# GassiusODude/spectral_analyzer

Hardware: NVIDIA B200
Metric: spectrogram Msamples/s (cf32, 1024-pt FFT) (higher is better)
Workload: dtype f32

## Files before the change

### spectral_analyzer_b200/csrc/engine.cu

```cuda
#include "engine_internal.h"

#include <algorithm>
#include <cmath>
#include <cstdarg>
#include <cstdio>
#include <cstdlib>
#include <cstring>
#include <cerrno>
#include <fcntl.h>
#include <sys/stat.h>
#include <unistd.h>

namespace sa {

#ifndef SA_LARGE_DUAL_DEFAULT
#define SA_LARGE_DUAL_DEFAULT 0
#endif
constexpr bool kLargeDualDefault = SA_LARGE_DUAL_DEFAULT != 0;
constexpr uint64_t kLargeDualWsMb = 48;

CopyPool::CopyPool(int workers) {
    for (int i = 0; i < workers; i++) threads_.emplace_back([this] { worker(); });
}
CopyPool::~CopyPool() {
// ... 265 lines not shown
    return fn;
}

int Engine::launch_spectrogram_large(const void* d_iq, uint64_t n_samples, const sa_spectrogram_params& p, int prec,
                                     const SpecArgs& base, void* d_out, cudaStream_t stream, int ws) {
    (void)d_iq; (void)n_samples; (void)d_out;
    const int dk = dtype_kind(p.dtype);
    const int win = (prec == SA_PREC_F64) ? 1 : (p.window != SA_WIN_RECT ? 1 : 0);
    const LargeKernelInfo* k = find_large_kernel(prec, (int)p.nfft, dk, win);
    if (!k) return set_error(SA_ERR_UNSUPPORTED, "no kernel for nfft %u precision %s dtype %d", p.nfft,
                             prec == SA_PREC_F64 ? "f64" : "f32", p.dtype);
    LargeArgs a;
    memset(&a, 0, sizeof(a));
    a.s = base;
    const SpecKernelInfo* k1 = find_spec_kernel(prec, k->n1, DK_CF32, 1, 0);
    const SpecKernelInfo* k2 = find_spec_kernel(prec, k->n2, DK_CF32, 1, 0);
    if (!k1 || !k2) return set_error(SA_ERR_UNSUPPORTED, "sub-transform plans %d / %d missing", k->n1, k->n2);
    int rc = twiddle_table(*k1, &a.s.twiddle);
    if (rc) return rc;
    rc = twiddle_table(*k2, &a.tw2);
    if (rc) return rc;
    rc = root_table((int)p.nfft, prec, &a.tw_n);
    if (rc) return rc;
    if (win) { rc = window_table(p.window, (int)p.nfft, prec, &a.s.window); if (rc) return rc; }
    const size_t elem = (prec == SA_PREC_F64) ? 16 : 8;
    const uint64_t per_frame = (uint64_t)p.nfft * elem;
    void* args[] = { &a };
    cudaError_t e;
    const char* onchip_env = getenv("SA_LARGE_ONCHIP");
    const bool use_onchip = onchip_env ? atoi(onchip_env) != 0 : false;
    const uint64_t iq_b = (uint64_t)sa_bytes_per_iq(p.dtype);
    const bool aligned = ((uintptr_t)d_iq % 16 == 0) && ((p.start_sample * iq_b) % 16 == 0) && ((p.hop * iq_b) % 16 == 0);
    if (k->fn_cluster && use_onchip && aligned) {
        auto it = occupancy.find(k->fn_cluster);
        int n_clusters = 0;
        cudaLaunchConfig_t cfg;
        memset(&cfg, 0, sizeof(cfg));
        cudaLaunchAttribute attr[1];
        attr[0].id = cudaLaunchAttributeClusterDimension;
        attr[0].val.clusterDim.x = kLargeCluster; attr[0].val.clusterDim.y = 1; attr[0].val.clusterDim.z = 1;
        cfg.blockDim = dim3(k->cta_cluster);
        cfg.dynamicSmemBytes = k->smem_cluster;
        cfg.stream = stream;
        cfg.attrs = attr; cfg.numAttrs = 1;
        if (it == occupancy.end()) {
            e = cudaFuncSetAttribute(k->fn_cluster, cudaFuncAttributeMaxDynamicSharedMemorySize, (int)k->smem_cluster);
            if (e != cudaSuccess) return cuda_fail(e, "on-chip four-step smem attribute");
            cfg.gridDim = dim3(kLargeCluster * num_sms);
            e = cudaOccupancyMaxActiveClusters(&n_clusters, k->fn_cluster, &cfg);
            if (e != cudaSuccess || n_clusters < 1) { cudaGetLastError(); n_clusters = 0; }
            occupancy[k->fn_cluster] = n_clusters;
        } else {
            n_clusters = it->second;
        }
        const uint64_t first_end = p.start_sample + p.nfft;
        const uint64_t n_read = n_samples >= first_end ? std::min<uint64_t>(p.n_frames, (n_samples - first_end) / p.hop + 1) : 0;
        CUtensorMap tmap;
        bool have_map = false;
        if (n_clusters > 0 && n_read > 0 && encode_tiled_fn()) {
            const cuuint64_t e8 = iq_b / 8;
            const cuuint64_t gdim[3] = { (cuuint64_t)k->n2 * e8, (cuuint64_t)k->n1, (cuuint64_t)n_read };
            const cuuint64_t gstr[2] = { (cuuint64_t)k->n2 * iq_b, (cuuint64_t)p.hop * iq_b };
            const cuuint32_t box[3] = { (cuuint32_t)(kLargeC * e8), (cuuint32_t)k->n1, 1 };
            const cuuint32_t estr[3] = { 1, 1, 1 };
            void* gaddr = (char*)const_cast<void*>(d_iq) + p.start_sample * iq_b;
            have_map = gstr[1] < (1ull << 40) &&
                       encode_tiled_fn()(&tmap, CU_TENSOR_MAP_DATA_TYPE_UINT64, 3, gaddr, gdim, gstr, box, estr, CU_TENSOR_MAP_INTERLEAVE_NONE,
                                         CU_TENSOR_MAP_SWIZZLE_NONE, CU_TENSOR_MAP_L2_PROMOTION_L2_256B,
                                         CU_TENSOR_MAP_FLOAT_OOB_FILL_NONE) == CUDA_SUCCESS;
        }
        if (have_map) {
            const uint64_t use = std::min<uint64_t>((uint64_t)n_clusters, p.n_frames);
            a.ws = nullptr;
#if SA_ONCHIP_PROF
            rc = ensure_scratch(ws, (size_t)use * kLargeCluster * 16 * sizeof(long long));
            if (rc) return rc;
            a.ws = scratch[ws];
#endif
            a.frame0 = 0;
            cfg.gridDim = dim3((unsigned)(use * kLargeCluster));
            void* cargs[] = { &a, &tmap };
            e = cudaLaunchKernelExC(&cfg, k->fn_cluster, cargs);
            if (e != cudaSuccess) return cuda_fail(e, "launch large_onchip_kernel");
            launches++;
// ... 138 lines not shown
            cudaLaunchConfig_t cfg;
            memset(&cfg, 0, sizeof(cfg));
            cfg.stream = st; cfg.attrs = attr; cfg.numAttrs = 1;
            cfg.gridDim = dim3(k->n2 / kLargeC, nf); cfg.blockDim = dim3(k->cta_cols); cfg.dynamicSmemBytes = k->smem_cols;
            e = cudaLaunchKernelExC(&cfg, k->fn_cols, args);
            if (e != cudaSuccess) return cuda_fail(e, "launch large_cols_kernel");
            cfg.gridDim = dim3(k->n1 / kLargeC, nf); cfg.blockDim = dim3(k->cta_rows); cfg.dynamicSmemBytes = k->smem_rows;
            e = cudaLaunchKernelExC(&cfg, k->fn_rows, args);
            if (e != cudaSuccess) return cuda_fail(e, "launch large_rows_kernel");
            launches += 2;
            continue;
        }
        e = cudaLaunchKernel(k->fn_cols, dim3(k->n2 / kLargeC, nf), dim3(k->cta_cols), args, k->smem_cols, st);
        if (e != cudaSuccess) return cuda_fail(e, "launch large_cols_kernel");
        e = cudaLaunchKernel(k->fn_rows, dim3(k->n1 / kLargeC, nf), dim3(k->cta_rows), args, k->smem_rows, st);
        if (e != cudaSuccess) return cuda_fail(e, "launch large_rows_kernel");
        launches += 2;
    }
    {
        static const char* const dkn[] = { "cf32", "ci16", "c8", "cf64" };
        char nm[160];
        snprintf(nm, sizeof(nm), "large_cols_kernel+large_rows_kernel<%s,%dx%d,%s,%s>", prec == SA_PREC_F64 ? "double" : "float",
                 k->n1, k->n2, dkn[dk], win ? "window" : "rect");
        last_kernel = nm;
    }
    if (dual) {
        e = cudaEventRecord(large_ev[ai][1], large_aux[ai]);
        if (e == cudaSuccess) e = cudaStreamWaitEvent(stream, large_ev[ai][1], 0);
        if (e != cudaSuccess) return cuda_fail(e, "four-step join");
    }
    return SA_OK;
}

int Engine::kernel_grid(const void* fn, int cta, size_t smem, int* blocks_per_sm) {
    auto it = occupancy.find(fn);
    if (it != occupancy.end()) { *blocks_per_sm = it->second; return SA_OK; }
    cudaError_t e = cudaFuncSetAttribute(fn, cudaFuncAttributeMaxDynamicSharedMemorySize, (int)smem);
    if (e != cudaSuccess) return cuda_fail(e, "cudaFuncSetAttribute(smem)");
    int nb = 0;
    e = cudaOccupancyMaxActiveBlocksPerMultiprocessor(&nb, fn, cta, smem);
    if (e != cudaSuccess) return cuda_fail(e, "occupancy query");
    if (nb < 1) return set_error(SA_ERR_CUDA, "kernel does not fit on an SM (smem %zu)", smem);
    occupancy[fn] = nb;
    *blocks_per_sm = nb;
    return SA_OK;
}

int dtype_kind(int dtype) {
    switch (dtype) {
        case SA_CF32: return DK_CF32;
        case SA_CI16: return DK_CI16;
        case SA_CU8:
        case SA_CI8:  return DK_C8;
        case SA_CF64: return DK_CF64;
        default:      return -1;
    }
}

void fill_load_params(LoadParams& lp, const void* base, int dtype, int big_endian) {
    lp.base = base;
    lp.swap = big_endian ? 1 : 0;
    lp.c8_flip = (dtype == SA_CI8) ? 0x80808080u : 0u;
    lp.c8_off = (dtype == SA_CI8) ? 1.0f : 127.5f / 128.0f;
    lp.c8_c = 256.0f + lp.c8_off;
}

static bool is_pow2(uint64_t x) { return x && !(x & (x - 1)); }

static bool strict_zero(const sa_spectrogram_params& p) {
    return p.strict_reference && (p.dtype == SA_CF64 || p.dtype == SA_DT_OTHER);
}
uint64_t spec_bytes_per_iq(const sa_spectrogram_params& p) {
    if (p.dtype == SA_DT_OTHER) return p.strict_reference ? 8 : 0;
    return (uint64_t)sa_bytes_per_iq(p.dtype);
}

// ... 93 lines not shown
    }
    if (p.nfft > 16384 || (prec == SA_PREC_F64 && p.nfft > 8192))
        return launch_spectrogram_large(d_iq, n_samples, p, prec, a, d_out, stream, ws);
    const uint64_t iq_b = (uint64_t)sa_bytes_per_iq(p.dtype);
    const bool aligned = ((uintptr_t)d_iq % 16 == 0) && ((p.start_sample * iq_b) % 16 == 0) && ((p.hop * iq_b) % 16 == 0);
    static const bool no_tma = getenv("SA_NO_TMA") != nullptr;
    static const bool no_mid = getenv("SA_NO_MID") != nullptr;
    const SpecKernelInfo* k = (aligned && !no_tma) ? find_spec_kernel(prec, (int)p.nfft, dk, win, 1) : nullptr;
    static const char* r64_env = getenv("SA_R64");
    const bool use_r64 = r64_env ? (strcmp(r64_env, "all") == 0) : (dk == DK_CF32 || dk == DK_CI16);
    if (!k && aligned && use_r64 && !pool_mode && prec == SA_PREC_F32 && p.nfft == 4096) k = find_spec_kernel(prec, 4096, dk, win, 4);
    const char* split_env = getenv("SA_SPLIT");
    const bool use_split = split_env ? atoi(split_env) != 0 : false;
    if (!k && aligned && use_split && !pool_mode && prec == SA_PREC_F32 && p.nfft == 2048) k = find_spec_kernel(prec, 2048, dk, win, 5);
    if (!k && aligned && !no_mid) {
        static const char* pf_env = getenv("SA_MID_PF");
        const bool pf = pf_env ? (strcmp(pf_env, "all") == 0) : (p.nfft != 8192);
        if (pf) k = find_spec_kernel(prec, (int)p.nfft, dk, win, 3);
        if (!k) k = find_spec_kernel(prec, (int)p.nfft, dk, win, 2);
    }
    if (!k) k = find_spec_kernel(prec, (int)p.nfft, dk, win, 0);
    if (!k) return set_error(SA_ERR_UNSUPPORTED, "no kernel for nfft %u precision %s dtype %d", p.nfft,
                             prec == SA_PREC_F64 ? "f64" : "f32", p.dtype);
    int rc;
    if (k->tma >= 2) {
        rc = mid_t1_table(k->n, &a.twiddle);
        if (rc) return rc;
        rc = root_table(k->n, prec, &a.aux);
    } else {
        rc = twiddle_table(*k, &a.twiddle);
    }
    if (rc) return rc;
    if (win) { rc = window_table(p.window, (int)p.nfft, prec, &a.window); if (rc) return rc; }
    int bps = 0;
    rc = kernel_grid(k->fn, k->cta, k->smem, &bps);
    if (rc) return rc;
    const long long n_blocks = ((long long)p.n_frames + k->fpc - 1) / k->fpc;
    const long long max_grid = (long long)bps * num_sms;
    const unsigned grid = (unsigned)std::min<long long>(n_blocks, max_grid);
    void* args[] = { &a };
    cudaError_t e = cudaLaunchKernel(k->fn, dim3(grid), dim3(k->cta), args, k->smem, stream);
    if (e != cudaSuccess) return cuda_fail(e, "launch spectrogram_kernel");
    launches++;
    {
        static const char* const fam[] = { "spectrogram_kernel", "spectrogram_tma_kernel", "spectrogram_mid_kernel",
                                           "spectrogram_mid_kernel(prefetch)", "spectrogram_r64_kernel", "spectrogram_split_kernel" };
        static const char* const dkn[] = { "cf32", "ci16", "c8", "cf64" };
        char nm[128];
        snprintf(nm, sizeof(nm), "%s<%s,%d,%s,%s>", fam[k->tma], prec == SA_PREC_F64 ? "double" : "float", k->n, dkn[k->dk],
                 k->win ? "window" : "rect");
        last_kernel = nm;
    }
    return SA_OK;
}

static CopyPool* make_copy_pool() {
    const char* ev = getenv("SA_COPY_THREADS");
    const unsigned hw = std::thread::hardware_concurrency();
    int n = ev ? atoi(ev) : (int)std::min(32u, std::max(2u, hw));
    return new CopyPool(std::max(1, n - 1));
}

void Engine::host_copy(void* dst, const void* src, size_t bytes) {
    if (bytes < (4u << 20)) { memcpy(dst, src, bytes); return; }
    if (!copy_pool) copy_pool = make_copy_pool();
    copy_pool->copy(dst, src, bytes);
}

bool Engine::host_read(void* dst, int fd, uint64_t off, size_t bytes) {
    if (!copy_pool) copy_pool = make_copy_pool();
    return copy_pool->read(dst, fd, off, bytes);
}

int Engine::ensure_staging(Slot& s, size_t in_bytes, size_t out_bytes) {
// ... 364 lines not shown
```

### spectral_analyzer_b200/csrc/fft_core.cuh

```cuda
#pragma once
#include <cuda_runtime.h>
#include <stdint.h>

#ifndef SA_WARPS_1WPF
#define SA_WARPS_1WPF 16
#endif
#ifndef SA_CTA_1WPF
#define SA_CTA_1WPF 512
#endif
#ifndef SA_CTA_F64
#define SA_CTA_F64 512
#endif
#ifndef SA_WIN_SMEM_MAX_TPF
#define SA_WIN_SMEM_MAX_TPF 128
#endif
#ifndef SA_TW_SMEM_MAX_TPF
#define SA_TW_SMEM_MAX_TPF 32
#endif
#ifndef SA_PACKED_SMALL_RADIX
#define SA_PACKED_SMALL_RADIX 0
#endif
#ifndef SA_TW_RECURRENCE
#define SA_TW_RECURRENCE 1
#endif
// ... 272 lines not shown
SA_PLAN(double,   64,  8, 2,  8,  8,  1, 1)
SA_PLAN(double,  128, 16, 2, 16,  8,  1, 1)
SA_PLAN(double,  256, 16, 2, 16, 16,  1, 1)
SA_PLAN(double,  512, 16, 3, 16, 16,  2, 1)
SA_PLAN(double, 1024, 16, 3, 16, 16,  4, 1)
SA_PLAN(double, 2048, 16, 3, 16, 16,  8, 1)
SA_PLAN(double, 4096, 16, 3, 16, 16, 16, 1)
SA_PLAN(double, 8192, 16, 4, 16, 16, 16, 2)
#undef SA_PLAN

template <typename T, int N> struct Geo {
    using PL = Plan<T, N>;
    static constexpr int P = PL::P;
    static constexpr int TPF = N / P;
    static constexpr int CTA = (sizeof(T) == 4 && TPF <= 32) ? SA_CTA_1WPF
                             : (sizeof(T) == 8 && TPF <= 32) ? SA_CTA_F64 : (TPF > 128 ? TPF : 128);
    static constexpr int FPC = CTA / TPF;
    static constexpr int MINB = (sizeof(T) == 4 && TPF <= 32) ? SA_WARPS_1WPF * 32 / CTA : 512 / CTA;
    static constexpr int WROW = P + 2;
    static constexpr bool WIN_SMEM = TPF <= SA_WIN_SMEM_MAX_TPF;
    static constexpr size_t WIN_BYTES = WIN_SMEM ? (size_t)TPF * WROW * sizeof(T) : 0;
    static constexpr int R0 = PL::radix(0);
    static constexpr int PADW = sizeof(T) == 4 ? 2 : 1;
    static constexpr int SM_ELEMS = N + (N / R0) * PADW;
    static constexpr size_t SMEM_BYTES = (size_t)FPC * SM_ELEMS * sizeof(cpx<T>);
    static constexpr bool TW_REC = SA_TW_RECURRENCE && sizeof(T) == 4 && PL::NP == 2 && PL::radix(1) == P;
    static constexpr bool TW_SMEM = TPF <= SA_TW_SMEM_MAX_TPF;
    static constexpr size_t TW_BYTES = TW_SMEM ? (size_t)(PL::NP - 1) * N * sizeof(cpx<T>) : 0;
    static constexpr size_t EXTRA_WIN_OFF = SMEM_BYTES + TW_BYTES;
    static constexpr int TW_ELEMS = (PL::NP - 1) * N;
    __host__ __device__ static constexpr int ns(int pass) { int r = 1; for (int i = 0; i < pass; i++) r *= PL::radix(i); return r; }
};

template <int R0, int PADW> __device__ __forceinline__ int pad_idx(int i) { return i + (i / R0) * PADW; }

template <int TPF, bool BSYNC = false> __device__ __forceinline__ void frame_sync() {
    if constexpr (TPF <= 32 && !BSYNC) __syncwarp(); else __syncthreads();
}

template <typename T, int N, int PASS, bool WIN, bool REC, bool BSYNC = false>
__device__ __forceinline__ void fft_pass(cpx<T> (&v)[Plan<T, N>::P], const int t, cpx<T>* __restrict__ sm,
                                         const cpx<T>* __restrict__ tw, const T* __restrict__ win,
                                         const TwSeed<T>& seed) {
    using G = Geo<T, N>;
    using PL = Plan<T, N>;
    constexpr int P = G::P, TPF = G::TPF, R = PL::radix(PASS), S = P / R, NS = G::ns(PASS);
    if constexpr (PASS == 0) {
        RadixAll<T, R, S, P, WIN ? MUL_REAL : MUL_NONE, false, 0>::run(v, win, nullptr, TPF, seed);
    } else {
        const TwPair<T>* twp = reinterpret_cast<const TwPair<T>*>(tw) + (size_t)(PASS - 1) * (N / 2) + t;
        if constexpr (REC && G::TW_REC) RadixAll<T, R, S, P, MUL_REC, false, 0>::run(v, nullptr, nullptr, TPF, seed);
        else RadixAll<T, R, S, P, MUL_CPX, G::TW_SMEM, 0>::run(v, nullptr, twp, TPF, seed);
    }
    if constexpr (PASS + 1 < PL::NP) {
        frame_sync<TPF, BSYNC>();
#pragma unroll
        for (int s = 0; s < S; s++) {
            const int j = t + TPF * s;
            const int base = (j / NS) * (NS * R) + (j % NS);
            if constexpr (NS == 1 && sizeof(T) == 4) {
                float4* dst = reinterpret_cast<float4*>(sm + pad_idx<G::R0, G::PADW>(base));
#pragma unroll
                for (int m = 0; m < R; m += 2)
                    dst[m / 2] = make_float4(v[s + m * S].x, v[s + m * S].y, v[s + (m + 1) * S].x, v[s + (m + 1) * S].y);
            } else {
#pragma unroll
                for (int m = 0; m < R; m++) sm[pad_idx<G::R0, G::PADW>(base + m * NS)] = v[s + m * S];
            }
        }
        frame_sync<TPF, BSYNC>();
#pragma unroll
        for (int q = 0; q < P; q++) v[q] = sm[pad_idx<G::R0, G::PADW>(t + TPF * q)];
    }
}

template <typename T, int N>
__device__ __forceinline__ TwSeed<T> load_tw_seed(const cpx<T>* __restrict__ tw, const int t) {
    using G = Geo<T, N>;
    TwSeed<T> s;
    s.om = mk2<T>((T)1, (T)0); s.oh = s.om;
    if constexpr (G::TW_REC) {
        const TwPair<T>* p = reinterpret_cast<const TwPair<T>*>(tw);
        s.om = ldg_tw<false>(p + 1 * G::TPF + t).lo;
        s.oh = ldg_tw<false>(p + 0 * G::TPF + t).hi;
    }
    return s;
}

template <typename T, int N, bool WIN, bool REC = false, bool BSYNC = false>
__device__ __forceinline__ void fft_frame(cpx<T> (&v)[Plan<T, N>::P], const int t, cpx<T>* __restrict__ sm,
                                          const cpx<T>* __restrict__ tw, const T* __restrict__ win,
                                          const TwSeed<T>& seed) {
    using PL = Plan<T, N>;
    fft_pass<T, N, 0, WIN, REC, BSYNC>(v, t, sm, tw, win, seed);
    if constexpr (PL::NP > 1) fft_pass<T, N, 1, WIN, REC, BSYNC>(v, t, sm, tw, win, seed);
    if constexpr (PL::NP > 2) fft_pass<T, N, 2, WIN, REC, BSYNC>(v, t, sm, tw, win, seed);
    if constexpr (PL::NP > 3) fft_pass<T, N, 3, WIN, REC, BSYNC>(v, t, sm, tw, win, seed);
}

}
```

### spectral_analyzer_b200/csrc/spectrogram_kernel.cuh

```cuda
#pragma once
#include "decode.cuh"

#ifndef SA_POOL_EPILOGUE
#define SA_POOL_EPILOGUE 1
#endif
#ifndef SA_STORE_STREAMING
#define SA_STORE_STREAMING 0
#endif

namespace sa {

enum { OUT_F32_DB = 0, OUT_F64_DB = 1, OUT_RGBA8 = 2 };
enum { DBM_MAG_1E10 = 0, DBM_POWER = 1 };

struct SpecArgs {
    LoadParams  lp;
    long long   n_samples;
    long long   start_sample;
    long long   hop;
    long long   n_frames;
    const void* window;
    const void* twiddle;
    const void* aux;
    void*       out;
    int         out_kind;
    int         db_mode;
    double      eof_fill;
    float       cmap_bias;
    float       inv_range;
    int         cmap;
    int         pool_mode;
    float       pool_eof;
    long long   pool_fpc;
    unsigned long long pool_magic;
};
__device__ __forceinline__ long long pool_column(const SpecArgs& a, long long frame) {
    return a.pool_magic ? (long long)__umul64hi((unsigned long long)frame, a.pool_magic) : frame;
}

__device__ __forceinline__ void pool_red(float* p, float v, int mode) {
    if (mode == 1) asm volatile("red.global.max.u32 [%0], %1;" ::"l"(p), "r"(__float_as_uint(v)) : "memory");
    else asm volatile("red.global.add.f32 [%0], %1;" ::"l"(p), "f"(v) : "memory");
}

#ifndef SA_F64_FAST_DB
#define SA_F64_FAST_DB 1
#endif
__device__ __forceinline__ float lg2_approx(float x) { float r; asm("lg2.approx.ftz.f32 %0, %1;" : "=f"(r) : "f"(x)); return r; }
__device__ __forceinline__ float sqrt_approx(float x) { float r; asm("sqrt.approx.ftz.f32 %0, %1;" : "=f"(r) : "f"(x)); return r; }

template <int MODE> __device__ __forceinline__ float to_db(float re, float im) {
    const float p = __fmaf_rn(re, re, im * im);
    if constexpr (MODE == DBM_MAG_1E10) return 6.02059991327962f * lg2_approx(sqrt_approx(p) + 1e-10f);
    return 3.01029995663981f * lg2_approx(p + 1e-20f);
}
template <int MODE> __device__ __forceinline__ double to_db(double re, double im) {
    if constexpr (MODE == DBM_MAG_1E10) return 20.0 * log10(sqrt(re * re + im * im) + 1e-10);
    return 10.0 * log10(re * re + im * im + 1e-20);
}

__device__ __forceinline__ float rcp_approx(float x) { float r; asm("rcp.approx.ftz.f32 %0, %1;" : "=f"(r) : "f"(x)); return r; }
__device__ __forceinline__ float rsqrt_approx(float x) { float r; asm("rsqrt.approx.ftz.f32 %0, %1;" : "=f"(r) : "f"(x)); return r; }
__device__ __forceinline__ float ltab_cell_mid(int k) { return __int_as_float(0x3f800000 | (k << 16) | 0x8000); }
__device__ __forceinline__ void f64_ltab_init(double* tab) {
    for (int k = threadIdx.x; k < 128; k += blockDim.x) tab[k] = -log2((double)rcp_approx(ltab_cell_mid(k)));
    __syncthreads();
}
// ... 238 lines not shown
            }
        }
        if (readable) {
            if (a.lp.swap) {
#pragma unroll
                for (int q = 0; q < P; q++) v[q] = Loader<T, DK>::template load<true>(a.lp, s0 + t + TPF * q);
            } else {
#pragma unroll
                for (int q = 0; q < P; q++) v[q] = Loader<T, DK>::template load<false>(a.lp, s0 + t + TPF * q);
            }
        } else {
#pragma unroll
            for (int q = 0; q < P; q++) v[q] = mk2<T>((T)0, (T)0);
        }

        fft_frame<T, N, WIN>(v, t, sm, tw, win, seed);

        if (!in_grid) continue;
        if (!readable) { store_fill<T, N>(a, frame, t); continue; }
        store_row<T, N>(a, frame, t, v, ltab);
    }
}

struct SpecKernelInfo {
    const void* fn;
    int prec;
    int n;
    int dk;
    int win;
    int cta;
    int fpc;
    int minb;
    size_t smem;
    int p;
    int np;
    int radix[4];
    int tma;
};

void register_spec_kernel(const SpecKernelInfo& k);

template <typename T, int N, int DK, bool WIN>
SpecKernelInfo make_spec_info(int prec) {
    using G = Geo<T, N>;
    using PL = Plan<T, N>;
    SpecKernelInfo k;
    k.fn = (const void*)&spectrogram_kernel<T, N, DK, WIN>;
    k.prec = prec; k.n = N; k.dk = DK; k.win = WIN ? 1 : 0;
    k.cta = G::CTA; k.fpc = G::FPC; k.minb = G::MINB; k.smem = G::SMEM_BYTES + G::TW_BYTES + (WIN ? G::WIN_BYTES : 0);
    k.p = G::P; k.np = PL::NP; k.tma = 0;
    for (int i = 0; i < 4; i++) k.radix[i] = PL::radix(i);
    return k;
}

}
```

### spectral_analyzer_b200/csrc/spectrogram_tma_kernel.cuh

```cuda
#pragma once
#include "spectrogram_kernel.cuh"

#ifndef SA_TMA_EVICT_LAST
#define SA_TMA_EVICT_LAST 0
#endif
#ifndef SA_TMA_BLOCKS_PER_STEP
#define SA_TMA_BLOCKS_PER_STEP 1
#endif

namespace sa {

__device__ __forceinline__ uint32_t smem_u32(const void* p) { return (uint32_t)__cvta_generic_to_shared(p); }

__device__ __forceinline__ void mbar_init(uint32_t bar, uint32_t count) {
    asm volatile("mbarrier.init.shared::cta.b64 [%0], %1;" ::"r"(bar), "r"(count));
}
__device__ __forceinline__ void mbar_expect_tx(uint32_t bar, uint32_t bytes) {
    asm volatile("mbarrier.arrive.expect_tx.shared::cta.b64 _, [%0], %1;" ::"r"(bar), "r"(bytes) : "memory");
}
__device__ __forceinline__ void mbar_wait(uint32_t bar, uint32_t parity) {
    asm volatile(
        "{\n\t.reg .pred p;\n\t"
        "WAIT_%=:\n\t"
        "mbarrier.try_wait.parity.shared::cta.b64 p, [%0], %1;\n\t"
        "@p bra DONE_%=;\n\t"
        "bra WAIT_%=;\n\t"
        "DONE_%=:\n\t}" ::"r"(bar), "r"(parity) : "memory");
}
__device__ __forceinline__ void tma_load_1d(uint32_t dst, const void* src, uint32_t bytes, uint32_t bar) {
#if SA_TMA_EVICT_LAST
    uint64_t pol;
    asm volatile("createpolicy.fractional.L2::evict_last.b64 %0, 1.0;" : "=l"(pol));
    asm volatile("cp.async.bulk.shared::cluster.global.mbarrier::complete_tx::bytes.L2::cache_hint [%0], [%1], %2, [%3], %4;"
                 ::"r"(dst), "l"(src), "r"(bytes), "r"(bar), "l"(pol) : "memory");
#else
    asm volatile("cp.async.bulk.shared::cluster.global.mbarrier::complete_tx::bytes [%0], [%1], %2, [%3];"
                 ::"r"(dst), "l"(src), "r"(bytes), "r"(bar) : "memory");
#endif
}
__device__ __forceinline__ void fence_proxy_async() { asm volatile("fence.proxy.async.shared::cta;" ::: "memory"); }

template <typename T, int N, int DK, bool WIN>
__global__ void __launch_bounds__(Geo<T, N>::CTA, Geo<T, N>::MINB)
spectrogram_tma_kernel(const SpecArgs a) {
    using G = Geo<T, N>;
    using LD = Loader<T, DK>;
    using raw_t = typename LD::raw_t;
    constexpr int P = G::P, TPF = G::TPF, FPC = G::FPC;
    static_assert(TPF == 32 && Plan<T, N>::NP == 2, "one warp per frame, two passes");
    constexpr uint32_t FRAME_BYTES = N * sizeof(raw_t);
    static_assert(FRAME_BYTES <= G::SM_ELEMS * sizeof(cpx<T>), "raw frame must fit the exchange buffer");
    extern __shared__ __align__(16) unsigned char smem_raw[];
    const int fl = threadIdx.x / TPF, t = threadIdx.x % TPF;
    cpx<T>* sm = reinterpret_cast<cpx<T>*>(smem_raw) + (size_t)fl * G::SM_ELEMS;
    const raw_t* raw = reinterpret_cast<const raw_t*>(sm);
    static_assert(G::TW_REC, "the TMA-staged kernel generates its pass-1 twiddles by recurrence");
    const cpx<T>* tw = reinterpret_cast<const cpx<T>*>(a.twiddle);
    const TwSeed<T> seed = load_tw_seed<T, N>(reinterpret_cast<const cpx<T>*>(a.twiddle), t);
    uint64_t* bars = reinterpret_cast<uint64_t*>(smem_raw + G::SMEM_BYTES + (WIN ? G::WIN_BYTES : 0));
    const uint32_t bar = smem_u32(&bars[fl]);
    const uint32_t dst = smem_u32(sm);

    T win_reg[G::WIN_SMEM ? 1 : P];
    const T* win = win_reg;
    if constexpr (WIN) win = setup_window<T, N>(a, smem_raw + G::SMEM_BYTES, win_reg, t);

    if (t == 0) mbar_init(bar, 1);
    __syncwarp();
    fence_proxy_async();

    const long long n_blocks = (a.n_frames + FPC - 1) / FPC;
    const char* base = reinterpret_cast<const char*>(a.lp.base);
    auto frame_of = [&](long long fb) { return fb * FPC + fl; };
    auto readable_f = [&](long long frame) {
        return frame < a.n_frames && (a.start_sample + frame * a.hop + N <= a.n_samples);
    };
    auto issue = [&](long long frame) {
        mbar_expect_tx(bar, FRAME_BYTES);
        tma_load_1d(dst, base + (a.start_sample + frame * a.hop) * (long long)sizeof(raw_t), FRAME_BYTES, bar);
    };

    constexpr long long K = SA_TMA_BLOCKS_PER_STEP;
    auto adv = [&](long long b) { return ((b + 1) % K != 0) ? b + 1 : b + 1 + ((long long)gridDim.x - 1) * K; };
    long long fb = (long long)blockIdx.x * K;
    if (fb < n_blocks && readable_f(frame_of(fb)) && t == 0) issue(frame_of(fb));
    uint32_t parity = 0;
    for (; fb < n_blocks; fb = adv(fb)) {
        const long long frame = frame_of(fb);
        const long long nfb = adv(fb);
        const long long next = frame_of(nfb);
        const bool next_readable = (nfb < n_blocks) && readable_f(next);
        if (frame >= a.n_frames) continue;
        if (!readable_f(frame)) {
            store_fill<T, N>(a, frame, t);
            if (next_readable && t == 0) issue(next);
            continue;
        }
        mbar_wait(bar, parity);
        parity ^= 1;
        cpx<T> v[P];
        if (a.lp.swap) {
#pragma unroll
            for (int q = 0; q < P; q++) v[q] = LD::template decode<true>(a.lp, raw[t + TPF * q]);
        } else {
#pragma unroll
            for (int q = 0; q < P; q++) v[q] = LD::template decode<false>(a.lp, raw[t + TPF * q]);
        }
        fft_pass<T, N, 0, WIN, true>(v, t, sm, tw, win, seed);
        __syncwarp();
        if (next_readable && t == 0) {
            fence_proxy_async();
            issue(next);
        }
        fft_pass<T, N, 1, WIN, true>(v, t, sm, tw, win, seed);
        store_row<T, N>(a, frame, t, v);
    }
}

template <typename T, int N, int DK, bool WIN>
SpecKernelInfo make_spec_tma_info(int prec) {
    SpecKernelInfo k = make_spec_info<T, N, DK, WIN>(prec);
    k.fn = (const void*)&spectrogram_tma_kernel<T, N, DK, WIN>;
    k.smem = Geo<T, N>::SMEM_BYTES + (WIN ? Geo<T, N>::WIN_BYTES : 0) + Geo<T, N>::FPC * sizeof(uint64_t);
    k.tma = 1;
    return k;
}

}
```

### spectral_analyzer_b200/csrc/engine_internal.h

```cpp
#pragma once
#include <cuda_runtime.h>
#include <atomic>
#include <condition_variable>
#include <map>
#include <mutex>
#include <string>
#include <thread>
#include <vector>

#include "../../include/sa_engine.h"
#include "spectrogram_tma_kernel.cuh"
#include "spectrogram_mid_kernel.cuh"
#include "large_fft_kernels.cuh"

namespace sa {

int set_error(int code, const char* fmt, ...);
int cuda_fail(cudaError_t e, const char* what);
const SpecKernelInfo* find_spec_kernel(int prec, int n, int dk, int win, int tma);
const LargeKernelInfo* find_large_kernel(int prec, int n, int dk, int win);
void host_window(int window_id, int n, std::vector<double>& w);
int dtype_kind(int dtype);
bool host_ptr_is_pinned(const void* p);
int check_spec_params(const sa_spectrogram_params* p, int* prec_out);
void fill_load_params(LoadParams& lp, const void* base, int dtype, int big_endian);
uint64_t spec_bytes_per_iq(const sa_spectrogram_params& p);

struct HostSource {
    const void* ptr = nullptr;
    int fd = -1;
    uint64_t file_off = 0;
};

struct AnalysisProfile {
    std::vector<double> taps;
    int delay_mode = SA_DELAY_CAUSAL;
    int length_mode = SA_LEN_FLOOR;
    int psd_scaling = SA_PSD_DENSITY;
    int psd_detrend = SA_DETREND_NONE;
    int psd_precision = SA_PREC_F32;
// ... 13 lines not shown
};

class CopyPool {
public:
    explicit CopyPool(int workers);
    ~CopyPool();
    struct Group { size_t outstanding = 0; };
    void copy(void* dst, const void* src, size_t bytes);
    bool read(void* dst, int fd, uint64_t off, size_t bytes);
    void start(void* dst, const void* src, size_t bytes, Group* g);
    void wait(Group* g);
private:
    void worker();
    void run(void* dst, const void* src, int fd, uint64_t off, size_t bytes);
    struct Job { char* dst; const char* src; size_t bytes; int fd; uint64_t off; Group* group; };
    std::atomic<bool> io_error_{false};
    std::vector<std::thread> threads_;
    std::mutex mu_;
    std::condition_variable cv_, done_cv_;
    std::vector<Job> queue_;
    bool stop_ = false;
};

struct Engine {
    int device = 0;
    int num_sms = 0;
    std::mutex mu;
    uint64_t launches = 0;
    std::string last_kernel;
    uint64_t chunk_bytes = 64ull << 20;
    std::map<uint64_t, void*> twiddles;
    std::map<uint64_t, void*> windows;
    std::map<uint64_t, void*> misc_tables;
    std::map<const void*, int> occupancy;
    std::vector<const void*> registered;
    Slot slots[kSlots];
    CopyPool* copy_pool = nullptr;
    void* scratch[kScratch] = {};
    size_t scratch_cap[kScratch] = {};
    cudaStream_t large_aux[4] = {};
    cudaEvent_t large_ev[4][2] = {};
    bool l2_persist_set = false; size_t l2_window_max = 0;
    AnalysisProfile profile;
    cudaStream_t dc_aux = nullptr;
    cudaEvent_t dc_ev[2] = {};
    cudaEvent_t dc_pipe_ev[4] = {};
    int dc_aux_prio = 0;
    void* h_plan = nullptr; size_t h_plan_cap = 0;
    cudaEvent_t plan_ev = nullptr;
    std::map<const void*, size_t> dc_smem_set;

    ~Engine();
    int twiddle_table(const SpecKernelInfo& k, const void** d_tab);
    int window_table(int window_id, int n, int prec, const void** d_tab);
    int kernel_grid(const void* fn, int cta, size_t smem, int* blocks_per_sm);
    int ensure_slot(Slot& s, size_t in_bytes, size_t out_bytes);
    int ensure_staging(Slot& s, size_t in_bytes, size_t out_bytes);
    void host_copy(void* dst, const void* src, size_t bytes);
    bool host_read(void* dst, int fd, uint64_t off, size_t bytes);
    int flush_pending(Slot& s);
    int ensure_scratch(int which, size_t bytes);
    int root_table(int n, int prec, const void** d_tab);
    int mid_t1_table(int n, const void** d_tab);
    int launch_spectrogram_large(const void* d_iq, uint64_t n_samples, const sa_spectrogram_params& p, int prec,
                                 const SpecArgs& base, void* d_out, cudaStream_t stream, int ws);
    int launch_spectrogram(const void* d_iq, uint64_t n_samples, const sa_spectrogram_params& p, int prec,
                           void* d_out, cudaStream_t stream, int ws = 2, int pool_mode = 0, uint64_t pool_fpc = 1);
    static bool can_pool(const sa_spectrogram_params& p, int prec) { return p.nfft <= 16384 && !(prec == SA_PREC_F64 && p.nfft > 8192); }
    int spectrogram_host(const HostSource& src, uint64_t iq_bytes, const sa_spectrogram_params& p, int prec, void* out);
};

}

struct sa_engine : public sa::Engine {};

#define ENGINE_ENTER(engine)                                                         \
    if (!(engine)) return set_error(SA_ERR_INVALID_ARG, "engine is NULL");            \
    std::lock_guard<std::mutex> lock_((engine)->mu);                                  \
    { cudaError_t e_ = cudaSetDevice((engine)->device);                               \
      if (e_ != cudaSuccess) return cuda_fail(e_, "cudaSetDevice"); }
```

Before: 336,500.

## Reuse overlapping half-frames via a three-slot TMA ring for 50% hop

When the hop is half the FFT size, each warp now processes a contiguous run of frames and keeps the previous frame's upper half in shared memory. Only the new half is loaded by TMA per frame, and the exchange buffer is split across ring slots. This is meant to halve global input traffic for the overlapped case. The cost is more shared memory per warp, an occupancy query sized for the larger layout, and extra slot-index logic.

```diff
diff --git a/spectral_analyzer_b200/csrc/engine.cu b/spectral_analyzer_b200/csrc/engine.cu
--- a/spectral_analyzer_b200/csrc/engine.cu
+++ b/spectral_analyzer_b200/csrc/engine.cu
@@ -712,14 +712,23 @@
     }
     if (rc) return rc;
     if (win) { rc = window_table(p.window, (int)p.nfft, prec, &a.window); if (rc) return rc; }
+    static const char* ring_env = getenv("SA_TMA_RING");
+    static const char* run_env = getenv("SA_TMA_RING_RUN");
+    const bool ring = k->tma == 1 && k->smem_ring && 2 * p.hop == p.nfft && !(ring_env && atoi(ring_env) == 0);
+    const size_t smem = ring ? k->smem_ring : k->smem;
     int bps = 0;
-    rc = kernel_grid(k->fn, k->cta, k->smem, &bps);
+    rc = kernel_grid(k->fn, k->cta, std::max(k->smem, k->smem_ring), &bps);
     if (rc) return rc;
     const long long n_blocks = ((long long)p.n_frames + k->fpc - 1) / k->fpc;
     const long long max_grid = (long long)bps * num_sms;
     const unsigned grid = (unsigned)std::min<long long>(n_blocks, max_grid);
+    if (ring) {
+        const long long warps = (long long)grid * k->fpc;
+        const long long run = run_env && atoll(run_env) > 0 ? atoll(run_env) : ((long long)p.n_frames + warps - 1) / warps;
+        a.ring = (int)std::min<long long>(run, 1 << 30);
+    }
     void* args[] = { &a };
-    cudaError_t e = cudaLaunchKernel(k->fn, dim3(grid), dim3(k->cta), args, k->smem, stream);
+    cudaError_t e = cudaLaunchKernel(k->fn, dim3(grid), dim3(k->cta), args, smem, stream);
     if (e != cudaSuccess) return cuda_fail(e, "launch spectrogram_kernel");
     launches++;
     {
diff --git a/spectral_analyzer_b200/csrc/fft_core.cuh b/spectral_analyzer_b200/csrc/fft_core.cuh
--- a/spectral_analyzer_b200/csrc/fft_core.cuh
+++ b/spectral_analyzer_b200/csrc/fft_core.cuh
@@ -328,7 +328,7 @@
     __host__ __device__ static constexpr int ns(int pass) { int r = 1; for (int i = 0; i < pass; i++) r *= PL::radix(i); return r; }
 };
 
-template <int R0, int PADW> __device__ __forceinline__ int pad_idx(int i) { return i + (i / R0) * PADW; }
+template <int R0, int PADW> __host__ __device__ __forceinline__ constexpr int pad_idx(int i) { return i + (i / R0) * PADW; }
 
 template <int TPF, bool BSYNC = false> __device__ __forceinline__ void frame_sync() {
     if constexpr (TPF <= 32 && !BSYNC) __syncwarp(); else __syncthreads();
@@ -337,10 +337,14 @@
 template <typename T, int N, int PASS, bool WIN, bool REC, bool BSYNC = false>
 __device__ __forceinline__ void fft_pass(cpx<T> (&v)[Plan<T, N>::P], const int t, cpx<T>* __restrict__ sm,
                                          const cpx<T>* __restrict__ tw, const T* __restrict__ win,
-                                         const TwSeed<T>& seed) {
+                                         const TwSeed<T>& seed, cpx<T>* sm_hi = nullptr) {
     using G = Geo<T, N>;
     using PL = Plan<T, N>;
     constexpr int P = G::P, TPF = G::TPF, R = PL::radix(PASS), S = P / R, NS = G::ns(PASS);
+    constexpr int XH = G::SM_ELEMS / 2;
+    static_assert(pad_idx<G::R0, G::PADW>(N / 2) == XH, "the exchange splits at the half frame");
+    cpx<T>* const smh = sm_hi ? sm_hi - XH : sm;
+    auto xp = [&](int i) { return (i < XH ? sm : smh) + i; };
     if constexpr (PASS == 0) {
         RadixAll<T, R, S, P, WIN ? MUL_REAL : MUL_NONE, false, 0>::run(v, win, nullptr, TPF, seed);
     } else {
@@ -355,18 +359,18 @@
             const int j = t + TPF * s;
             const int base = (j / NS) * (NS * R) + (j % NS);
             if constexpr (NS == 1 && sizeof(T) == 4) {
-                float4* dst = reinterpret_cast<float4*>(sm + pad_idx<G::R0, G::PADW>(base));
+                float4* dst = reinterpret_cast<float4*>(xp(pad_idx<G::R0, G::PADW>(base)));
 #pragma unroll
                 for (int m = 0; m < R; m += 2)
                     dst[m / 2] = make_float4(v[s + m * S].x, v[s + m * S].y, v[s + (m + 1) * S].x, v[s + (m + 1) * S].y);
             } else {
 #pragma unroll
-                for (int m = 0; m < R; m++) sm[pad_idx<G::R0, G::PADW>(base + m * NS)] = v[s + m * S];
+                for (int m = 0; m < R; m++) *xp(pad_idx<G::R0, G::PADW>(base + m * NS)) = v[s + m * S];
             }
         }
         frame_sync<TPF, BSYNC>();
 #pragma unroll
-        for (int q = 0; q < P; q++) v[q] = sm[pad_idx<G::R0, G::PADW>(t + TPF * q)];
+        for (int q = 0; q < P; q++) v[q] = (q < P / 2 ? sm : smh)[pad_idx<G::R0, G::PADW>(t + TPF * q)];
     }
 }
 
diff --git a/spectral_analyzer_b200/csrc/spectrogram_kernel.cuh b/spectral_analyzer_b200/csrc/spectrogram_kernel.cuh
--- a/spectral_analyzer_b200/csrc/spectrogram_kernel.cuh
+++ b/spectral_analyzer_b200/csrc/spectrogram_kernel.cuh
@@ -33,6 +33,7 @@
     float       pool_eof;
     long long   pool_fpc;
     unsigned long long pool_magic;
+    int         ring;
 };
 __device__ __forceinline__ long long pool_column(const SpecArgs& a, long long frame) {
     return a.pool_magic ? (long long)__umul64hi((unsigned long long)frame, a.pool_magic) : frame;
@@ -337,6 +338,7 @@
     int fpc;
     int minb;
     size_t smem;
+    size_t smem_ring = 0;
     int p;
     int np;
     int radix[4];
diff --git a/spectral_analyzer_b200/csrc/spectrogram_tma_kernel.cuh b/spectral_analyzer_b200/csrc/spectrogram_tma_kernel.cuh
--- a/spectral_analyzer_b200/csrc/spectrogram_tma_kernel.cuh
+++ b/spectral_analyzer_b200/csrc/spectrogram_tma_kernel.cuh
@@ -1,5 +1,6 @@
 #pragma once
 #include "spectrogram_kernel.cuh"
+#include "tma_ring.cuh"
 
 #ifndef SA_TMA_EVICT_LAST
 #define SA_TMA_EVICT_LAST 0
@@ -40,6 +41,16 @@
 }
 __device__ __forceinline__ void fence_proxy_async() { asm volatile("fence.proxy.async.shared::cta;" ::: "memory"); }
 
+template <typename T, int N> struct TmaSmem {
+    using G = Geo<T, N>;
+    static constexpr size_t SLOT = (size_t)G::SM_ELEMS / 2 * sizeof(cpx<T>);
+    static constexpr size_t RING_BUF = (size_t)G::FPC * RING_SLOTS * SLOT;
+    static constexpr size_t bytes(bool ring, bool win) {
+        return ring ? (size_t)ring_smem_bytes(G::FPC, SLOT, win ? G::WIN_BYTES : 0)
+                    : G::SMEM_BYTES + (win ? G::WIN_BYTES : 0) + G::FPC * sizeof(uint64_t);
+    }
+};
+
 template <typename T, int N, int DK, bool WIN>
 __global__ void __launch_bounds__(Geo<T, N>::CTA, Geo<T, N>::MINB)
 spectrogram_tma_kernel(const SpecArgs a) {
@@ -57,24 +68,89 @@
     static_assert(G::TW_REC, "the TMA-staged kernel generates its pass-1 twiddles by recurrence");
     const cpx<T>* tw = reinterpret_cast<const cpx<T>*>(a.twiddle);
     const TwSeed<T> seed = load_tw_seed<T, N>(reinterpret_cast<const cpx<T>*>(a.twiddle), t);
-    uint64_t* bars = reinterpret_cast<uint64_t*>(smem_raw + G::SMEM_BYTES + (WIN ? G::WIN_BYTES : 0));
+    const size_t buf_bytes = a.ring ? TmaSmem<T, N>::RING_BUF : G::SMEM_BYTES;
+    uint64_t* bars = reinterpret_cast<uint64_t*>(smem_raw + buf_bytes + (WIN ? G::WIN_BYTES : 0));
     const uint32_t bar = smem_u32(&bars[fl]);
     const uint32_t dst = smem_u32(sm);
 
     T win_reg[G::WIN_SMEM ? 1 : P];
     const T* win = win_reg;
-    if constexpr (WIN) win = setup_window<T, N>(a, smem_raw + G::SMEM_BYTES, win_reg, t);
+    if constexpr (WIN) win = setup_window<T, N>(a, smem_raw + buf_bytes, win_reg, t);
 
     if (t == 0) mbar_init(bar, 1);
     __syncwarp();
     fence_proxy_async();
 
-    const long long n_blocks = (a.n_frames + FPC - 1) / FPC;
     const char* base = reinterpret_cast<const char*>(a.lp.base);
-    auto frame_of = [&](long long fb) { return fb * FPC + fl; };
     auto readable_f = [&](long long frame) {
         return frame < a.n_frames && (a.start_sample + frame * a.hop + N <= a.n_samples);
     };
+    auto transform = [&](const long long frame, const raw_t* raw_lo, const raw_t* raw_hi, cpx<T>* x_lo, cpx<T>* x_hi,
+                         const bool next, auto&& issue_next) {
+        cpx<T> v[P];
+        if (a.lp.swap) {
+#pragma unroll
+            for (int q = 0; q < P; q++) v[q] = LD::template decode<true>(a.lp, q < P / 2 ? raw_lo[t + TPF * q] : raw_hi[t + TPF * (q - P / 2)]);
+        } else {
+#pragma unroll
+            for (int q = 0; q < P; q++) v[q] = LD::template decode<false>(a.lp, q < P / 2 ? raw_lo[t + TPF * q] : raw_hi[t + TPF * (q - P / 2)]);
+        }
+        fft_pass<T, N, 0, WIN, true>(v, t, x_lo, tw, win, seed, x_hi);
+        __syncwarp();
+        if (next && t == 0) {
+            fence_proxy_async();
+            issue_next();
+        }
+        fft_pass<T, N, 1, WIN, true>(v, t, x_lo, tw, win, seed, x_hi);
+        store_row<T, N>(a, frame, t, v);
+    };
+    uint32_t parity = 0;
+
+    if (a.ring) {
+        constexpr uint32_t HALF_BYTES = FRAME_BYTES / 2;
+        constexpr uint32_t SLOT_BYTES = TmaSmem<T, N>::SLOT;
+        static_assert(HALF_BYTES <= SLOT_BYTES && SLOT_BYTES % 16 == 0, "a raw half fits one slot");
+        unsigned char* slots = smem_raw + (size_t)fl * RING_SLOTS * SLOT_BYTES;
+        auto slot = [&](int s) { return slots + s * SLOT_BYTES; };
+        auto half = [&](long long frame, int h) {
+            return base + (a.start_sample + frame * a.hop) * (long long)sizeof(raw_t) + h * HALF_BYTES;
+        };
+        const long long W = (long long)gridDim.x * FPC, R = a.ring;
+        RingPos p = ring_first((long long)blockIdx.x * FPC + fl, R, a.n_frames);
+        if (p.frame < a.n_frames && readable_f(p.frame) && t == 0) {
+            mbar_expect_tx(bar, 2 * HALF_BYTES);
+            tma_load_1d(smem_u32(slot(0)), half(p.frame, 0), HALF_BYTES, bar);
+            tma_load_1d(smem_u32(slot(1)), half(p.frame, 1), HALF_BYTES, bar);
+        }
+        int s = 0;
+        while (p.frame < a.n_frames) {
+            const RingPos q = ring_succ(p, W, R, a.n_frames);
+            const bool next = q.frame < a.n_frames && readable_f(q.frame);
+            if (!readable_f(p.frame)) {
+                store_fill<T, N>(a, p.frame, t);
+            } else {
+                const RingStep st = ring_step(s);
+                mbar_wait(bar, parity);
+                parity ^= 1;
+                transform(p.frame, reinterpret_cast<const raw_t*>(slot(st.raw_lo)), reinterpret_cast<const raw_t*>(slot(st.raw_hi)),
+                          reinterpret_cast<cpx<T>*>(slot(st.x_lo)), reinterpret_cast<cpx<T>*>(slot(st.x_hi)), next, [&] {
+                              if (q.frame == p.frame + 1) {
+                                  mbar_expect_tx(bar, HALF_BYTES);
+                              } else {
+                                  mbar_expect_tx(bar, 2 * HALF_BYTES);
+                                  tma_load_1d(smem_u32(slot(st.copy_lo)), half(q.frame, 0), HALF_BYTES, bar);
+                              }
+                              tma_load_1d(smem_u32(slot(st.copy_hi)), half(q.frame, 1), HALF_BYTES, bar);
+                          });
+            }
+            p = q;
+            s = ring_next(s);
+        }
+        return;
+    }
+
+    const long long n_blocks = (a.n_frames + FPC - 1) / FPC;
+    auto frame_of = [&](long long fb) { return fb * FPC + fl; };
     auto issue = [&](long long frame) {
         mbar_expect_tx(bar, FRAME_BYTES);
         tma_load_1d(dst, base + (a.start_sample + frame * a.hop) * (long long)sizeof(raw_t), FRAME_BYTES, bar);
@@ -84,7 +160,6 @@
     auto adv = [&](long long b) { return ((b + 1) % K != 0) ? b + 1 : b + 1 + ((long long)gridDim.x - 1) * K; };
     long long fb = (long long)blockIdx.x * K;
     if (fb < n_blocks && readable_f(frame_of(fb)) && t == 0) issue(frame_of(fb));
-    uint32_t parity = 0;
     for (; fb < n_blocks; fb = adv(fb)) {
         const long long frame = frame_of(fb);
         const long long nfb = adv(fb);
@@ -98,22 +173,7 @@
         }
         mbar_wait(bar, parity);
         parity ^= 1;
-        cpx<T> v[P];
-        if (a.lp.swap) {
-#pragma unroll
-            for (int q = 0; q < P; q++) v[q] = LD::template decode<true>(a.lp, raw[t + TPF * q]);
-        } else {
-#pragma unroll
-            for (int q = 0; q < P; q++) v[q] = LD::template decode<false>(a.lp, raw[t + TPF * q]);
-        }
-        fft_pass<T, N, 0, WIN, true>(v, t, sm, tw, win, seed);
-        __syncwarp();
-        if (next_readable && t == 0) {
-            fence_proxy_async();
-            issue(next);
-        }
-        fft_pass<T, N, 1, WIN, true>(v, t, sm, tw, win, seed);
-        store_row<T, N>(a, frame, t, v);
+        transform(frame, raw, raw + N / 2, sm, sm + G::SM_ELEMS / 2, next_readable, [&] { issue(next); });
     }
 }
 
@@ -121,7 +181,9 @@
 SpecKernelInfo make_spec_tma_info(int prec) {
     SpecKernelInfo k = make_spec_info<T, N, DK, WIN>(prec);
     k.fn = (const void*)&spectrogram_tma_kernel<T, N, DK, WIN>;
-    k.smem = Geo<T, N>::SMEM_BYTES + (WIN ? Geo<T, N>::WIN_BYTES : 0) + Geo<T, N>::FPC * sizeof(uint64_t);
+    k.smem = TmaSmem<T, N>::bytes(false, WIN);
+    k.smem_ring = TmaSmem<T, N>::bytes(true, WIN);
+    static_assert(TmaSmem<T, N>::bytes(true, WIN) <= 232448, "the ring layout fits the opt-in shared memory of an SM");
     k.tma = 1;
     return k;
 }
diff --git a/spectral_analyzer_b200/csrc/tma_ring.cuh b/spectral_analyzer_b200/csrc/tma_ring.cuh
--- /dev/null
+++ b/spectral_analyzer_b200/csrc/tma_ring.cuh
@@ -0,0 +1,45 @@
+#pragma once
+#ifndef __CUDACC__
+#define __host__
+#define __device__
+#define __forceinline__ inline
+#endif
+
+namespace sa {
+
+constexpr int RING_SLOTS = 3;
+
+struct RingPos { long long frame, end, run; };
+__host__ __device__ __forceinline__ RingPos ring_run_pos(long long run, long long R, long long n_frames) {
+    RingPos p;
+    p.run = run;
+    p.frame = run * R;
+    p.end = p.frame + R < n_frames ? p.frame + R : n_frames;
+    return p;
+}
+__host__ __device__ __forceinline__ RingPos ring_first(long long g, long long R, long long n_frames) {
+    return ring_run_pos(g, R, n_frames);
+}
+__host__ __device__ __forceinline__ RingPos ring_succ(const RingPos& p, long long W, long long R, long long n_frames) {
+    if (p.frame + 1 < p.end) { RingPos q = p; q.frame = p.frame + 1; return q; }
+    return ring_run_pos(p.run + W, R, n_frames);
+}
+
+__host__ __device__ __forceinline__ int ring_next(int s) { return s == RING_SLOTS - 1 ? 0 : s + 1; }
+
+struct RingStep { int raw_lo, raw_hi, x_lo, x_hi, copy_lo, copy_hi; };
+__host__ __device__ __forceinline__ RingStep ring_step(int s) {
+    const int s1 = ring_next(s), s2 = ring_next(s1);
+    RingStep r;
+    r.raw_lo = s; r.raw_hi = s1;
+    r.x_lo = s; r.x_hi = s2;
+    r.copy_lo = s1; r.copy_hi = s2;
+    return r;
+}
+
+__host__ __device__ constexpr unsigned long long ring_smem_bytes(int warps, unsigned long long slot_bytes,
+                                                                 unsigned long long win_bytes) {
+    return (unsigned long long)warps * RING_SLOTS * slot_bytes + win_bytes + (unsigned long long)warps * 8ull;
+}
+
+}
```

Result: slower. 330,800, median of 6 (-1.7%).

## Reuse overlapping half-frames via per-warp TMA ring when hop is half the FFT

Applied to the files above, without the earlier changes.

When hop equals nfft/2, each warp now processes a contiguous range of frames and keeps a three-slot half-frame ring in shared memory, so each new frame needs only one half-frame TMA load instead of a full frame. This halves global input traffic for 50%-overlap spectrograms and uses a different shared-memory size, which may change occupancy. The occupancy cache is keyed by function and smem size to support the two launch configurations. Work distribution changes from strided blocks to contiguous per-warp frame ranges, which may affect load balance and store locality.

```diff
diff --git a/spectral_analyzer_b200/csrc/engine.cu b/spectral_analyzer_b200/csrc/engine.cu
--- a/spectral_analyzer_b200/csrc/engine.cu
+++ b/spectral_analyzer_b200/csrc/engine.cu
@@ -321,7 +321,7 @@
     const uint64_t iq_b = (uint64_t)sa_bytes_per_iq(p.dtype);
     const bool aligned = ((uintptr_t)d_iq % 16 == 0) && ((p.start_sample * iq_b) % 16 == 0) && ((p.hop * iq_b) % 16 == 0);
     if (k->fn_cluster && use_onchip && aligned) {
-        auto it = occupancy.find(k->fn_cluster);
+        auto it = occupancy.find({k->fn_cluster, k->smem_cluster});
         int n_clusters = 0;
         cudaLaunchConfig_t cfg;
         memset(&cfg, 0, sizeof(cfg));
@@ -338,7 +338,7 @@
             cfg.gridDim = dim3(kLargeCluster * num_sms);
             e = cudaOccupancyMaxActiveClusters(&n_clusters, k->fn_cluster, &cfg);
             if (e != cudaSuccess || n_clusters < 1) { cudaGetLastError(); n_clusters = 0; }
-            occupancy[k->fn_cluster] = n_clusters;
+            occupancy[{k->fn_cluster, k->smem_cluster}] = n_clusters;
         } else {
             n_clusters = it->second;
         }
@@ -543,16 +543,16 @@
     return SA_OK;
 }
 
-int Engine::kernel_grid(const void* fn, int cta, size_t smem, int* blocks_per_sm) {
-    auto it = occupancy.find(fn);
+int Engine::kernel_grid(const void* fn, int cta, size_t smem, int* blocks_per_sm, size_t smem_limit) {
+    auto it = occupancy.find({fn, smem});
     if (it != occupancy.end()) { *blocks_per_sm = it->second; return SA_OK; }
-    cudaError_t e = cudaFuncSetAttribute(fn, cudaFuncAttributeMaxDynamicSharedMemorySize, (int)smem);
+    cudaError_t e = cudaFuncSetAttribute(fn, cudaFuncAttributeMaxDynamicSharedMemorySize, (int)std::max(smem, smem_limit));
     if (e != cudaSuccess) return cuda_fail(e, "cudaFuncSetAttribute(smem)");
     int nb = 0;
     e = cudaOccupancyMaxActiveBlocksPerMultiprocessor(&nb, fn, cta, smem);
     if (e != cudaSuccess) return cuda_fail(e, "occupancy query");
     if (nb < 1) return set_error(SA_ERR_CUDA, "kernel does not fit on an SM (smem %zu)", smem);
-    occupancy[fn] = nb;
+    occupancy[{fn, smem}] = nb;
     *blocks_per_sm = nb;
     return SA_OK;
 }
@@ -712,14 +712,18 @@
     }
     if (rc) return rc;
     if (win) { rc = window_table(p.window, (int)p.nfft, prec, &a.window); if (rc) return rc; }
+    static const char* ring_env = getenv("SA_TMA_RING");
+    static const bool no_ring = ring_env && atoi(ring_env) == 0;
+    a.tma_ring = (k->tma == 1 && 2 * p.hop == p.nfft && !no_ring) ? 1 : 0;
+    const size_t smem = a.tma_ring ? k->smem_ring : k->smem;
     int bps = 0;
-    rc = kernel_grid(k->fn, k->cta, k->smem, &bps);
+    rc = kernel_grid(k->fn, k->cta, smem, &bps, std::max(k->smem, k->smem_ring));
     if (rc) return rc;
     const long long n_blocks = ((long long)p.n_frames + k->fpc - 1) / k->fpc;
     const long long max_grid = (long long)bps * num_sms;
     const unsigned grid = (unsigned)std::min<long long>(n_blocks, max_grid);
     void* args[] = { &a };
-    cudaError_t e = cudaLaunchKernel(k->fn, dim3(grid), dim3(k->cta), args, k->smem, stream);
+    cudaError_t e = cudaLaunchKernel(k->fn, dim3(grid), dim3(k->cta), args, smem, stream);
     if (e != cudaSuccess) return cuda_fail(e, "launch spectrogram_kernel");
     launches++;
     {
diff --git a/spectral_analyzer_b200/csrc/engine_internal.h b/spectral_analyzer_b200/csrc/engine_internal.h
--- a/spectral_analyzer_b200/csrc/engine_internal.h
+++ b/spectral_analyzer_b200/csrc/engine_internal.h
@@ -6,6 +6,7 @@
 #include <mutex>
 #include <string>
 #include <thread>
+#include <utility>
 #include <vector>
 
 #include "../../include/sa_engine.h"
@@ -85,7 +86,7 @@
     std::map<uint64_t, void*> twiddles;
     std::map<uint64_t, void*> windows;
     std::map<uint64_t, void*> misc_tables;
-    std::map<const void*, int> occupancy;
+    std::map<std::pair<const void*, size_t>, int> occupancy;
     std::vector<const void*> registered;
     Slot slots[kSlots];
     CopyPool* copy_pool = nullptr;
@@ -106,7 +107,7 @@
     ~Engine();
     int twiddle_table(const SpecKernelInfo& k, const void** d_tab);
     int window_table(int window_id, int n, int prec, const void** d_tab);
-    int kernel_grid(const void* fn, int cta, size_t smem, int* blocks_per_sm);
+    int kernel_grid(const void* fn, int cta, size_t smem, int* blocks_per_sm, size_t smem_limit = 0);
     int ensure_slot(Slot& s, size_t in_bytes, size_t out_bytes);
     int ensure_staging(Slot& s, size_t in_bytes, size_t out_bytes);
     void host_copy(void* dst, const void* src, size_t bytes);
diff --git a/spectral_analyzer_b200/csrc/spectrogram_kernel.cuh b/spectral_analyzer_b200/csrc/spectrogram_kernel.cuh
--- a/spectral_analyzer_b200/csrc/spectrogram_kernel.cuh
+++ b/spectral_analyzer_b200/csrc/spectrogram_kernel.cuh
@@ -33,6 +33,7 @@
     float       pool_eof;
     long long   pool_fpc;
     unsigned long long pool_magic;
+    int         tma_ring;
 };
 __device__ __forceinline__ long long pool_column(const SpecArgs& a, long long frame) {
     return a.pool_magic ? (long long)__umul64hi((unsigned long long)frame, a.pool_magic) : frame;
@@ -341,6 +342,7 @@
     int np;
     int radix[4];
     int tma;
+    size_t smem_ring = 0;
 };
 
 void register_spec_kernel(const SpecKernelInfo& k);
diff --git a/spectral_analyzer_b200/csrc/spectrogram_tma_kernel.cuh b/spectral_analyzer_b200/csrc/spectrogram_tma_kernel.cuh
--- a/spectral_analyzer_b200/csrc/spectrogram_tma_kernel.cuh
+++ b/spectral_analyzer_b200/csrc/spectrogram_tma_kernel.cuh
@@ -40,37 +40,96 @@
 }
 __device__ __forceinline__ void fence_proxy_async() { asm volatile("fence.proxy.async.shared::cta;" ::: "memory"); }
 
+template <typename T, int N, bool WIN>
+struct TmaGeo {
+    using G = Geo<T, N>;
+    static constexpr size_t BAR_OFF = WIN ? G::WIN_BYTES : 0;
+    static constexpr size_t BUF_OFF = BAR_OFF + G::FPC * sizeof(uint64_t);
+    static constexpr int HALF = G::SM_ELEMS / 2;
+    static_assert(N / 2 + (N / 2 / G::R0) * G::PADW == HALF, "the exchange must split into two slots");
+    static constexpr size_t FULL_BYTES = BUF_OFF + (size_t)G::FPC * G::SM_ELEMS * sizeof(cpx<T>);
+    static constexpr size_t RING_BYTES = BUF_OFF + (size_t)G::FPC * 3 * HALF * sizeof(cpx<T>);
+    static_assert(BAR_OFF % 128 == 0 && BUF_OFF % 128 == 0 && (HALF * sizeof(cpx<T>)) % 128 == 0, "bank alignment");
+};
+
 template <typename T, int N, int DK, bool WIN>
 __global__ void __launch_bounds__(Geo<T, N>::CTA, Geo<T, N>::MINB)
 spectrogram_tma_kernel(const SpecArgs a) {
     using G = Geo<T, N>;
+    using TG = TmaGeo<T, N, WIN>;
     using LD = Loader<T, DK>;
     using raw_t = typename LD::raw_t;
-    constexpr int P = G::P, TPF = G::TPF, FPC = G::FPC;
+    constexpr int P = G::P, TPF = G::TPF, FPC = G::FPC, HALF = TG::HALF;
     static_assert(TPF == 32 && Plan<T, N>::NP == 2, "one warp per frame, two passes");
-    constexpr uint32_t FRAME_BYTES = N * sizeof(raw_t);
+    constexpr uint32_t FRAME_BYTES = N * sizeof(raw_t), HALF_BYTES = FRAME_BYTES / 2;
     static_assert(FRAME_BYTES <= G::SM_ELEMS * sizeof(cpx<T>), "raw frame must fit the exchange buffer");
+    static_assert(HALF_BYTES % 16 == 0 && HALF_BYTES <= HALF * sizeof(cpx<T>), "raw half frame must fit a ring slot");
     extern __shared__ __align__(16) unsigned char smem_raw[];
     const int fl = threadIdx.x / TPF, t = threadIdx.x % TPF;
-    cpx<T>* sm = reinterpret_cast<cpx<T>*>(smem_raw) + (size_t)fl * G::SM_ELEMS;
-    const raw_t* raw = reinterpret_cast<const raw_t*>(sm);
+    cpx<T>* const buf = reinterpret_cast<cpx<T>*>(smem_raw + TG::BUF_OFF);
     static_assert(G::TW_REC, "the TMA-staged kernel generates its pass-1 twiddles by recurrence");
     const cpx<T>* tw = reinterpret_cast<const cpx<T>*>(a.twiddle);
     const TwSeed<T> seed = load_tw_seed<T, N>(reinterpret_cast<const cpx<T>*>(a.twiddle), t);
-    uint64_t* bars = reinterpret_cast<uint64_t*>(smem_raw + G::SMEM_BYTES + (WIN ? G::WIN_BYTES : 0));
-    const uint32_t bar = smem_u32(&bars[fl]);
-    const uint32_t dst = smem_u32(sm);
+    const uint32_t bar = smem_u32(smem_raw + TG::BAR_OFF + fl * sizeof(uint64_t));
 
     T win_reg[G::WIN_SMEM ? 1 : P];
     const T* win = win_reg;
-    if constexpr (WIN) win = setup_window<T, N>(a, smem_raw + G::SMEM_BYTES, win_reg, t);
+    if constexpr (WIN) win = setup_window<T, N>(a, smem_raw, win_reg, t);
 
     if (t == 0) mbar_init(bar, 1);
     __syncwarp();
     fence_proxy_async();
+    const char* base = reinterpret_cast<const char*>(a.lp.base);
 
+    if (a.tma_ring) {
+        constexpr long long HOP = N / 2;
+        const long long W = (long long)gridDim.x * FPC, g = (long long)blockIdx.x * FPC + fl;
+        const long long f0 = g * a.n_frames / W, f1 = (g + 1) * a.n_frames / W;
+        const long long avail = a.n_samples - a.start_sample - N;
+        const long long fr = avail < 0 ? f0 : max(f0, min(f1, avail / HOP + 1));
+        cpx<T>* const s0 = buf + (size_t)fl * 3 * HALF;
+        const char* src = base + (a.start_sample + f0 * HOP) * (long long)sizeof(raw_t);
+        if (f0 < fr && t == 0) {
+            mbar_expect_tx(bar, FRAME_BYTES);
+            tma_load_1d(smem_u32(s0 + 2 * HALF), src, HALF_BYTES, bar);
+            tma_load_1d(smem_u32(s0), src + HALF_BYTES, HALF_BYTES, bar);
+        }
+        int lo = 2 * HALF;
+        uint32_t parity = 0;
+        for (long long f = f0; f < fr; f++) {
+            mbar_wait(bar, parity);
+            parity ^= 1;
+            const raw_t* raw_lo = reinterpret_cast<const raw_t*>(s0 + lo);
+            const raw_t* raw_hi = reinterpret_cast<const raw_t*>(s0 + (2 * HALF - lo));
+            cpx<T> v[P];
+            if (a.lp.swap) {
+#pragma unroll
+                for (int q = 0; q < P; q++) v[q] = LD::template decode<true>(a.lp, q < P / 2 ? raw_lo[t + TPF * q] : raw_hi[t + TPF * (q - P / 2)]);
+            } else {
+#pragma unroll
+                for (int q = 0; q < P; q++) v[q] = LD::template decode<false>(a.lp, q < P / 2 ? raw_lo[t + TPF * q] : raw_hi[t + TPF * (q - P / 2)]);
+            }
+            cpx<T>* const sm = s0 + (lo >> 1);
+            fft_pass<T, N, 0, WIN, true>(v, t, sm, tw, win, seed);
+            __syncwarp();
+            if (f + 1 < fr && t == 0) {
+                fence_proxy_async();
+                mbar_expect_tx(bar, HALF_BYTES);
+                tma_load_1d(smem_u32(s0 + lo), src + FRAME_BYTES, HALF_BYTES, bar);
+            }
+            fft_pass<T, N, 1, WIN, true>(v, t, sm, tw, win, seed);
+            store_row<T, N>(a, f, t, v);
+            src += HALF_BYTES;
+            lo = 2 * HALF - lo;
+        }
+        for (long long f = fr; f < f1; f++) store_fill<T, N>(a, f, t);
+        return;
+    }
+
+    cpx<T>* sm = buf + (size_t)fl * G::SM_ELEMS;
+    const raw_t* raw = reinterpret_cast<const raw_t*>(sm);
+    const uint32_t dst = smem_u32(sm);
     const long long n_blocks = (a.n_frames + FPC - 1) / FPC;
-    const char* base = reinterpret_cast<const char*>(a.lp.base);
     auto frame_of = [&](long long fb) { return fb * FPC + fl; };
     auto readable_f = [&](long long frame) {
         return frame < a.n_frames && (a.start_sample + frame * a.hop + N <= a.n_samples);
@@ -121,7 +180,8 @@
 SpecKernelInfo make_spec_tma_info(int prec) {
     SpecKernelInfo k = make_spec_info<T, N, DK, WIN>(prec);
     k.fn = (const void*)&spectrogram_tma_kernel<T, N, DK, WIN>;
-    k.smem = Geo<T, N>::SMEM_BYTES + (WIN ? Geo<T, N>::WIN_BYTES : 0) + Geo<T, N>::FPC * sizeof(uint64_t);
+    k.smem = TmaGeo<T, N, WIN>::FULL_BYTES;
+    k.smem_ring = TmaGeo<T, N, WIN>::RING_BYTES;
     k.tma = 1;
     return k;
 }
```

After: 331,400 before, 341,200 after (median of 6 runs). +3.0%, better.
